# byu-magicc/VI-EKF

Hardware: AMD Instinct MI355X
Metric: EKF steps/sec (IMU-rate propagate + N_feat updates), batch=1024, N_feat=50 (higher is better)
Workload: dtype f64

## Files before the change

### vi_ekf_amd/csrc/viekf_fused_lds.hpp

```cpp
#pragma once
#include <cstddef>

#include "viekf_instance_rows.hpp"

#if defined(__HIPCC__)
#define VIEKF_HD __host__ __device__
#else
#define VIEKF_HD
#endif

namespace viekf {

constexpr int RES_FMT_LOAD_PACKED = 1, RES_FMT_STORE_PACKED = 2, RES_FMT_P_ONLY = 4;
constexpr int launch_pack(bool prop, int kp, int fmt, int dbg) { return (prop ? (1 | (kp << 16)) : 0) | (fmt << 1) | ((dbg & 0xff) << 8); }
constexpr int launch_prop(int w) { return w & 1; }
constexpr int launch_fmt(int w) { return (w >> 1) & 7; }
constexpr int launch_dbg(int w) { return (w >> 8) & 0xff; }
constexpr int launch_kp(int w) { return (w >> 16) > 0 ? (w >> 16) : 1; }

enum : unsigned { SM_RES1 = 1, SM_RES2 = 2, SM_TILE = 4, SM_TILE_PAIR = 8 };
struct SmWords {
  const char* name;
  int at, count;
  bool is_int;
  bool zero;
  unsigned live;
  const char* writer;
  const char* reader;
};

namespace res_sm {
enum { MB_H0, MB_H1, MB_H2, MB_H3, MB_R0, MB_R1, MB_S0, MB_S1, MB_S2, MB_S3, MB_GATE, MB_FIELDS };
constexpr int MB_STRIDE = 16;
constexpr int mbox(int mb) { return MB_STRIDE * mb; }
constexpr int mbox_seq(int mb) { return 32 + mb; }
constexpr int fix_word(int role, int par) { return (role == 2 ? 36 : 40) + par; }
constexpr int DT = 42;
constexpr int nan_word(int role, int phase) { return (role == 2 ? 52 : 44) + phase % 3; }
constexpr int gate_word(int phase) { return 50 + (phase & 1); }
constexpr int CTRL_WORDS = 64;
constexpr int SQRTQU = CTRL_WORDS, QXB = SQRTQU + 6;
constexpr int len(bool staged) { return staged ? QXB + 16 : CTRL_WORDS; }
inline constexpr SmWords kWords[] = {
    {"mailbox 0", mbox(0), MB_FIELDS, false, false, SM_RES2, "the service wave that holds the feature (send)", "the other service wave (recv)"},
    {"mailbox 1", mbox(1), MB_FIELDS, false, false, SM_RES2, "the service wave that holds the feature (send)", "the other service wave (recv)"},
    {"mailbox sequence numbers", mbox_seq(0), 2, true, true, SM_RES2, "send", "recv (polls)"},
    {"fix mailbox non-empty, body wave", fix_word(2, 0), 2, false, true, SM_RES2, "service role 2", "workers (fix_word)"},
    {"fix mailbox non-empty", fix_word(0, 0), 2, false, true, SM_RES1 | SM_RES2, "service role 0 / 1", "workers (fix_word)"},
    {"dt", DT, 1, false, false, SM_RES1 | SM_RES2, "prologue; service (next propagate of several)", "service, res_prop_setup"},
    {"NaN guard", nan_word(0, 0), 3, false, true, SM_RES1 | SM_RES2, "service role 0 / 1 (gain_rows)", "workers; service role 2"},
    {"(dead: once the count of published raw columns)", 49, 1, true, true, 0, "nobody", "nobody"},
    {"gate verdict", gate_word(0), 2, false, true, SM_RES1 | SM_RES2, "service role 0 / 1 (gain_rows)", "workers"},
    {"NaN guard, body wave", nan_word(2, 0), 3, false, true, SM_RES2, "service role 2 (gain_rows)", "workers; service role 1"},
    {"sqrt(Qu)", SQRTQU, 6, false, false, SM_RES1 | SM_RES2, "prologue", "res_prop_setup"},
    {"Qx of the body rows", QXB, 16, false, false, SM_RES1 | SM_RES2, "prologue", "res_prop_body"},
};
}

namespace tile_sm {
enum { MB_G00, MB_G01, MB_G11, MB_SKIP, MB_FIELDS };
constexpr int MB_STRIDE = 8;
constexpr int mbox(int mb) { return MB_STRIDE * mb; }
constexpr int fix_word(int par) { return 40 + par; }
constexpr int DT = 42;
constexpr int nan_word(int phase) { return 44 + phase % 3; }
constexpr int TRIPS = 60;
constexpr int CTRL_WORDS = 64;
constexpr int len() { return CTRL_WORDS; }
inline constexpr SmWords kWords[] = {
    {"mailbox 0", mbox(0), MB_FIELDS, false, false, SM_TILE | SM_TILE_PAIR, "service (publish)", "workers"},
    {"mailbox 1", mbox(1), MB_FIELDS, false, false, SM_TILE | SM_TILE_PAIR, "service (publish)", "workers"},
    {"fix mailbox non-empty", fix_word(0), 2, false, true, SM_TILE | SM_TILE_PAIR, "service", "workers"},
    {"dt", DT, 1, false, false, SM_TILE | SM_TILE_PAIR, "prologue; service (next propagate of several)", "service, res_prop_setup"},
    {"NaN in the column pair", nan_word(0), 3, false, true, SM_TILE | SM_TILE_PAIR, "workers (set; clear two phases ahead)", "workers, service"},
    {"updates that will run", TRIPS, 1, false, false, SM_TILE_PAIR, "prologue", "both halves of a paired workgroup"},
};
}

template <int NWD>
constexpr unsigned long long sm_zero_mask(const SmWords (&words)[NWD]) {
  unsigned long long m = 0;
  for (int i = 0; i < NWD; i++)
    if (words[i].zero)
      for (int w = words[i].at; w < words[i].at + words[i].count; w++) m |= 1ull << w;
  return m;
}

constexpr std::size_t kBodyCtxBytes = 440;
constexpr int ZK = 9;
constexpr int ZS = 26;

VIEKF_HD inline int res_mcap(int N) { return N > 64 ? 80 : 64; }

constexpr bool res_batched_loads(int RB, int NW) { return NW != 7 && RB != 8; }

struct ResLds {
  int xs, Kt, Wt, Praw, lam, sm, fixadd, fixset, Z, phiff, Abb, Gb, Phibb, Mbb, Gdb, Pbb, T16, xdb, ctx, Pbc, PhibbT, Pd, PsiP, Pi, Xi, AvG, Lbc, mslot, mseq, mz, mR, img_len, total;
  VIEKF_HD ResLds(int N, int n, int nxs, bool staged, std::size_t ctx_bytes) {
    const int nf = 3 * N;
    int o = 0;
    auto take = [&](int cnt) { int r = o; o += (cnt + 1) & ~1; return r; };
    xs = take(nxs);
    lam = take(n);
    sm = take(res_sm::len(staged));
    fixadd = take(2 * (N > 0 ? N : 1)); fixset = take(2 * (N > 0 ? N : 1));
    Z = take(nf * ZS > 4 * n ? nf * ZS : 4 * n);
    phiff = take(9 * (N > 0 ? N : 1));
    const int u0 = o;
    Abb = take(256); Gb = take(96); Phibb = take(256); PhibbT = take(256); Gdb = take(96); T16 = take(256);
    PsiP = take(ZK * 16); Pi = take(ZK * ZK); Xi = take(ZK * 16); AvG = take(18);
    const int uprop = o;
    o = u0;
    Kt = take(2 * n); Wt = take(2 * n);
    Praw = take(4 * n > 256 ? 4 * n : 256);
    Pd = take(4 * (N > 0 ? N : 1));
    if (uprop > o) o = uprop;
    img_len = o - Z;
    Mbb = take(256); Pbb = take(256);
    xdb = take(16);
    ctx = take((int)((ctx_bytes + 7) / 8));
    Pbc = take(nf * 16);
    Lbc = take(48);
    const int mc = res_mcap(N);
    mslot = take(mc / 2); mseq = take(mc); mz = take(2 * mc); mR = take(4 * mc);
    total = o;
  }
};

VIEKF_HD inline int tile_nt(int N) { return 1 + (N + 4) / 5; }

struct TileLds {
  int xs, lam, sm, fixadd, fixset, Z, phiff, Abb, Gb, Phibb, PhibbT, Gdb, T16, PsiP, Pi, Xi, AvG, Cb, Eb, Pd, Mbb, Pbb, xdb, ctx, Pbc,
      mslot, mseq, mz, mR, total;
  VIEKF_HD TileLds(int N, int n, int nxs, std::size_t ctx_bytes) {
    const int nf = 3 * N, NQ = 16 * tile_nt(N);
    int o = 0;
    auto take = [&](int cnt) { int r = o; o += (cnt + 1) & ~1; return r; };
    xs = take(nxs);
    lam = take(n);
    sm = take(tile_sm::len());
    fixadd = take(2 * (N > 0 ? N : 1)); fixset = take(2 * (N > 0 ? N : 1));
    Z = take(nf * ZS);
    phiff = take(9 * (N > 0 ? N : 1));
    const int u0 = o;
    Abb = take(256); Gb = take(96); Phibb = take(256); PhibbT = take(256); Gdb = take(96); T16 = take(256);
    PsiP = take(ZK * 16); Pi = take(ZK * ZK); Xi = take(ZK * 16); AvG = take(18);
    const int uprop = o;
    o = u0;
    Cb = take(4 * NQ);
    Eb = take(4 * NQ);
    Pd = take(4 * (N > 0 ? N : 1));
    if (uprop > o) o = uprop;
    Mbb = take(256); Pbb = take(256);
    xdb = take(16);
    ctx = take((int)((ctx_bytes + 7) / 8));
    Pbc = take(nf * 16);
    const int mc = res_mcap(N);
    mslot = take(mc / 2); mseq = take(mc); mz = take(2 * mc); mR = take(4 * mc);
    total = o;
  }
  VIEKF_HD int pair_word(int half, int w) const { return half * total + sm + w; }
};

}
```

### vi_ekf_amd/csrc/viekf_host.hpp

```cpp
#pragma once
#include <map>
#include <string>
#include <vector>

namespace viekf {

typedef std::map<std::string, std::string> YamlMap;
bool yaml_parse_file(const std::string& path, YamlMap& out, std::string& err);
bool yaml_get_doubles(const YamlMap& m, const std::string& key, double* out, int count, std::string& err);
bool yaml_get_string(const YamlMap& m, const std::string& key, std::string& out, std::string& err);
int set_last_error(int code, const std::string& msg);
bool build_resmap(int N, int RB, int NWV, std::vector<int>& map, int* used_slots = nullptr);

inline int cov_ld(int num_features) {
  const int n = 16 + 3 * num_features;
#ifdef VIEKF_LD_PAD_ALL
  return (n + 15) & ~15;
#endif
  return num_features > 77 ? (n + 15) & ~15 : (n + 1) & ~1;
}

}
```

### vi_ekf_amd/csrc/viekf_resident_worker.hpp

```cpp
#pragma once
#include "viekf_resident_prop.hpp"

namespace viekf {


struct StoreChunk { int f0, f1, rb, h; };
__device__ __forceinline__ bool store_chunk_at(int f0, int N, int n, int img_len, StoreChunk& c) {
  if (f0 >= N) return false;
  c.f0 = f0;
  c.rb = (16 + 3 * f0) & ~1;
  c.h = ((n + 1) & ~1) - c.rb;
  c.f1 = min(N, f0 + max(1, img_len / (3 * c.h)));
  return true;
}
template <int T>
__device__ __forceinline__ void res_store_chunk(const StreamArgs& a, const ResShared& S, const StoreChunk& c, int tid) {
  const int n = S.n, ld = a.ld;
  double* P = a.P_out + S.so * n * ld;
  const double* img = S.Z;
  const int ncol = 3 * (c.f1 - c.f0), lane = tid & 63, w = tid >> 6;
  constexpr int NWV = T / 64;
  if ((n & 1) == 0) {
#pragma unroll 2
    for (int col = w; col < ncol; col += NWV) {
      const int j = 16 + 3 * c.f0 + col;
      const double* src = img + col * c.h - c.rb;
      for (int i0 = c.rb; i0 < n; i0 += 256) {
        double2 v[2];
#pragma unroll
        for (int u = 0; u < 2; u++) v[u] = lds_ld2(src + min(i0 + 2 * (lane + 64 * u), n - 2));
#pragma unroll
        for (int u = 0; u < 2; u++) {
          const int i = i0 + 2 * (lane + 64 * u);
          if (i < n && i + 1 >= j) *reinterpret_cast<double2*>(P + i + (long)j * ld) = v[u];
        }
      }
    }
  } else {
#pragma unroll 2
    for (int col = w; col < ncol; col += NWV) {
      const int j = 16 + 3 * c.f0 + col;
      const double* src = img + col * c.h - c.rb;
      for (int i = c.rb + lane; i < n; i += 64)
        if (i >= j) P[i + (long)j * ld] = src[i];
    }
  }
}

template <int RB, int TW>
__device__ __forceinline__ void res_store_packed(double* img, const double (&pb)[RB][9], const double* Pbc, const double* Pbb,
                                                 int N, int t) {
  constexpr ResPack K(0, RB, TW / 64);
  v2f64* dst = reinterpret_cast<v2f64*>(img) + t;
#pragma unroll
  for (int p = 0; p < K.npair; p++) {
    v2f64 v;
    v.x = pb[(2 * p) / 9][(2 * p) % 9];
    v.y = pb[(2 * p + 1) / 9][(2 * p + 1) % 9];
    dst[p * TW] = v;
  }
  if ((9 * RB) & 1) img[K.single + t] = pb[RB - 1][8];
  v2f64* gc = reinterpret_cast<v2f64*>(img + K.pbc);
  for (int e = t; e < 24 * N; e += TW) gc[e] = *reinterpret_cast<const v2f64*>(Pbc + 2 * e);
  v2f64* gb = reinterpret_cast<v2f64*>(img + K.pbc + 48 * N);
  for (int e = t; e < 128; e += TW) gb[e] = *reinterpret_cast<const v2f64*>(Pbb + 2 * e);
}
__device__ __forceinline__ void res_body_items(const ResShared& S, const double* kP, bool run, int id, int nthreads,
                                               int first, int last, int slot2, double* rawdst) {
  const double* wP = kP + 2 * S.n;
  double* Pbc = S.Pbc;
  const int j2 = ((first + id) & 7) * 2;
  double2 cw0 = {}, cw1 = {}, cl[3] = {};
  if (run) {
    cw0 = lds_ld2(wP + 2 * j2);
    cw1 = lds_ld2(wP + 2 * j2 + 2);
#pragma unroll
    for (int q = 0; q < 3; q++) cl[q] = lds_ld2(S.Lbc + 16 * q + j2);
  }
#pragma unroll 1
  for (int item = first + id; item < last; item += nthreads) {
    const int g = item >> 3;
    double2 cpv[3];
#pragma unroll
    for (int q = 0; q < 3; q++) cpv[q] = lds_ld2(Pbc + (3 * g + q) * 16 + j2);
    if (run) {
      double2 cki[3];
#pragma unroll
      for (int q = 0; q < 3; q++) cki[q] = lds_ld2(kP + 2 * (16 + 3 * g + q));
#pragma unroll
      for (int q = 0; q < 3; q++) {
        cpv[q].x = fma(-cl[q].x, fma(cki[q].y, cw0.y, cki[q].x * cw0.x), cpv[q].x);
        cpv[q].y = fma(-cl[q].y, fma(cki[q].y, cw1.y, cki[q].x * cw1.x), cpv[q].y);
        *reinterpret_cast<double2*>(Pbc + (3 * g + q) * 16 + j2) = cpv[q];
      }
    }
    if (g == slot2) {
      double* st = rawdst + 2 * j2;
      *reinterpret_cast<double2*>(st) = make_double2(cpv[0].x, cpv[1].x);
      *reinterpret_cast<double2*>(st + 2) = make_double2(cpv[0].y, cpv[1].y);
    }
  }
}
template <int RB, int TW, bool MP, int T = TW + 64, bool ZU = false, bool BL = true>
__device__ __forceinline__ void res_worker(const StreamArgs& a, const ResShared& S, int tid) {
  constexpr bool SU = res_setup_under_load(RB, TW / 64, MP);
  constexpr int RR = res_rotating_reads(RB, TW / 64, MP, ZU);
  const int N = S.N, n = S.n, ld = a.ld, nf = S.nf, len = S.len;
  double* P = a.P + S.si * n * ld;
  const int tid_ = tid;
  constexpr int NWV = TW / 64;
  const DevParams& prm = a.prm(uniform_filter(S.b));
  double* Pbc = S.Pbc;
  double* Pbb = S.Pbb;
  const int* __restrict__ resmap = a.resmap;
  auto blk = [&](const int (&w)[RB], int t, int ia, int& I, int& J) -> bool {
    return res_word_blk(BL ? w[ia] : resmap[ia * TW + t], I, J);
  };
  const bool own_diag = tid_ < N;

  double pb[RB][9];
  const bool ldp = (S.fmt & RES_FMT_LOAD_PACKED) != 0;
  double Lff[9];
  bool partial_su = false;
  if (SU) {
    const double lf[3] = {a.lam(uniform_filter(S.b))[16], a.lam(uniform_filter(S.b))[17], a.lam(uniform_filter(S.b))[18]};
#pragma unroll
    for (int r = 0; r < 3; r++)
#pragma unroll
      for (int s = 0; s < 3; s++) Lff[r * 3 + s] = uniform_f64(prm.use_partial_update ? (lf[s] + lf[r] - lf[r] * lf[s]) : 1.0);
    partial_su = prm.use_partial_update != 0;
  }
  if (ldp) {
    const int t = opaque(tid_);
    constexpr ResPack K(0, RB, TW / 64);
    const v2f64* gc = reinterpret_cast<const v2f64*>(P + K.pbc);
    for (int e = t; e < 24 * N; e += TW) *reinterpret_cast<v2f64*>(Pbc + 2 * e) = gc[e];
    const v2f64* gb = reinterpret_cast<const v2f64*>(P + K.pbc + 48 * N);
    for (int e = t; e < 128; e += TW) *reinterpret_cast<v2f64*>(Pbb + 2 * e) = gb[e];
  }
  if (SU) {
    for (int e = tid; !ldp && e < nf * 16; e += TW) {
      const int k = e / nf, row = e - k * nf;
      Pbc[row * 16 + k] = P[(16 + row) + (long)k * ld];
    }
    for (int e = tid; !ldp && e < 256; e += TW) {
      const int r = e & 15, c = e >> 4;
      Pbb[r * 16 + c] = P[max(r, c) + (long)min(r, c) * ld];
    }
  }
  int ws[SU ? RB : 1];
  double qs[3];
  {
    const int tq = opaque(tid_);
    int ew[RB];
    if (BL) res_words<RB, TW>(resmap, tq, ew);
    if (SU) {
#pragma unroll
      for (int ia = 0; ia < RB; ia++) ws[ia] = ew[ia];
      if (S.do_prop) {
#pragma unroll
        for (int r = 0; r < 3; r++) qs[r] = a.qx(uniform_filter(S.b))[16 + 3 * min(tq, N - 1) + r];
      }
    }
#pragma unroll
    for (int ia = 0; ia < (SU ? RB / 4 : RB); ia++) {
      int I, J;
      blk(ew, tq, ia, I, J);
      const bool up = I < J;
      const int br = 16 + 3 * (up ? J : I), bc = 16 + 3 * (up ? I : J);
      const unsigned cbase = (unsigned)(br + bc * ld);
      const unsigned base = ldp ? 2u * (unsigned)tq : cbase, base1 = ldp ? (unsigned)tq : cbase;
#pragma unroll
      for (int s = 0; s < 3; s++)
#pragma unroll
        for (int r = 0; r < 3; r++) {
          const int rr = (I == J) ? max(r, s) : (up ? s : r), cc = (I == J) ? min(r, s) : (up ? r : s);
          constexpr ResPack K(0, RB, TW / 64);
          const int q = ia * 9 + r * 3 + s;
          const unsigned offp = (unsigned)K.elem(q, 0), offc = (unsigned)(rr + cc * ld);
          pb[ia][r * 3 + s] = P[((q < 2 * K.npair) ? base : base1) + (ldp ? offp : offc)];
        }
    }
    for (int e = tid; !SU && !ldp && e < nf * 16; e += TW) {
      const int k = e / nf, row = e - k * nf;
      Pbc[row * 16 + k] = P[(16 + row) + (long)k * ld];
    }
    for (int e = tid; !SU && !ldp && e < 256; e += TW) {
      const int r = e & 15, c = e >> 4;
      Pbb[r * 16 + c] = P[max(r, c) + (long)min(r, c) * ld];
    }
  }

  auto issue_chunk = [&](auto kc) {
    constexpr int k = decltype(kc)::value + 1, lo = RB * k / 4, hi = RB * (k + 1) / 4;
    const int tq = opaque(tid_);
#pragma unroll
    for (int ia = lo; ia < hi; ia++) {
      int I, J;
      res_word_blk(ws[SU ? ia : 0], I, J);
      const bool up = I < J;
      const int br = 16 + 3 * (up ? J : I), bc = 16 + 3 * (up ? I : J);
      const unsigned cbase = (unsigned)(br + bc * ld);
      const unsigned base = ldp ? 2u * (unsigned)tq : cbase, base1 = ldp ? (unsigned)tq : cbase;
#pragma unroll
      for (int s = 0; s < 3; s++)
#pragma unroll
        for (int r = 0; r < 3; r++) {
          const int rr = (I == J) ? max(r, s) : (up ? s : r), cc = (I == J) ? min(r, s) : (up ? r : s);
          constexpr ResPack K(0, RB, TW / 64);
          const int q = ia * 9 + r * 3 + s;
          const unsigned offp = (unsigned)K.elem(q, 0), offc = (unsigned)(rr + cc * ld);
          pb[ia][r * 3 + s] = P[((q < 2 * K.npair) ? base : base1) + (ldp ? offp : offc)];
        }
    }
  };

  auto sym_diag = [&]() {
    if (own_diag) { pb[0][3] = pb[0][1]; pb[0][6] = pb[0][2]; pb[0][7] = pb[0][5]; }
  };
  if (!SU) {
    sym_diag();
    const double lf[3] = {a.lam(uniform_filter(S.b))[16], a.lam(uniform_filter(S.b))[17], a.lam(uniform_filter(S.b))[18]};
#pragma unroll
    for (int r = 0; r < 3; r++)
#pragma unroll
      for (int s = 0; s < 3; s++) Lff[r * 3 + s] = uniform_f64(prm.use_partial_update ? (lf[s] + lf[r] - lf[r] * lf[s]) : 1.0);
  }
  const bool partial = SU ? partial_su : prm.use_partial_update != 0;
  int par = 0;
  constexpr int NSV = (T - TW) / 64;
  auto fix_word = [&](int mb) -> double { return (NSV > 1) ? S.sm[res_sm::fix_word(1, mb)] + S.sm[res_sm::fix_word(2, mb)] : S.sm[res_sm::fix_word(0, mb)]; };
  RES_STAMP(S, tid == 0, 64);
  __syncthreads();
  RES_STAMP(S, tid == 0, 65);

  const int nkp = MP ? S.kp : 1;
  int eu[RB];
  if (S.do_prop)
   for (int kp = 0; kp < nkp; kp++) {
    const int tk = MP ? opaque(tid) : tid;
    const double* Z = S.Z; double* phiff = S.phiff;
    int ep[RB];
    double qd[3];
    if (SU) {
#pragma unroll
      for (int ia = 0; ia < RB; ia++) ep[ia] = ws[SU ? ia : 0];
#pragma unroll
      for (int r = 0; r < 3; r++) qd[r] = qs[r];
    } else if (BL) {
      const int tq = opaque(tid_);
      res_words<RB, TW>(resmap, tq, ep);
#pragma unroll
      for (int r = 0; r < 3; r++) qd[r] = a.qx(uniform_filter(S.b))[16 + 3 * min(tq, N - 1) + r];
    }
    if (MP || !BL) res_prop_setup<TW>(a, S, tk);
    else if (SU) res_prop_setup<TW, true, decltype(issue_chunk), res_service_setup(RB, TW / 64, MP)>(a, S, tk, issue_chunk);
    else res_prop_setup<TW, true>(a, S, tk);
    RES_STAMP(S, tid == 0, 66);
    __syncthreads();
    RES_STAMP(S, tid == 0, 67);
#ifdef VIEKF_STAMPS
    asm volatile("s_waitcnt vmcnt(0)" ::: "memory");
#endif
    RES_STAMP(S, tid == 0, 74);
    if (SU) sym_diag();

#pragma unroll
    for (int ia = 0; ia < RB; ia++) {
      const int tq = BL ? 0 : opaque(tid_);
      int I, J;
      const bool v = blk(ep, tq, ia, I, J);
      const double* fj = phiff + 9 * J;
#pragma unroll
      for (int r = 0; r < 3; r++) {
        const double p0 = pb[ia][r * 3 + 0], p1 = pb[ia][r * 3 + 1], p2 = pb[ia][r * 3 + 2];
#pragma unroll
        for (int s = 0; s < 3; s++) pb[ia][r * 3 + s] = p0 * fj[s * 3 + 0] + p1 * fj[s * 3 + 1] + p2 * fj[s * 3 + 2];
      }
      const double* fi = phiff + 9 * I;
#pragma unroll
      for (int s = 0; s < 3; s++) {
        const double p0 = pb[ia][0 * 3 + s], p1 = pb[ia][1 * 3 + s], p2 = pb[ia][2 * 3 + s];
#pragma unroll
        for (int r = 0; r < 3; r++) pb[ia][r * 3 + s] = fi[r * 3 + 0] * p0 + fi[r * 3 + 1] * p1 + fi[r * 3 + 2] * p2;
      }
      if (BL) {
        if (ia == 0 && own_diag) { pb[0][0] += qd[0]; pb[0][4] += qd[1]; pb[0][8] += qd[2]; }
      } else if (v && I == J) {
        pb[ia][0] += a.qx(uniform_filter(S.b))[16 + 3 * I + 0];
        pb[ia][4] += a.qx(uniform_filter(S.b))[16 + 3 * I + 1];
        pb[ia][8] += a.qx(uniform_filter(S.b))[16 + 3 * I + 2];
      }
      __builtin_amdgcn_sched_barrier(0);
      if (RB > 4) {
#pragma unroll
        for (int e = 0; e < 9; e++) asm volatile("" : "+v"(pb[ia][e]));
      }
      group_fence<(RB > 4)>();
    }
    RES_STAMP(S, tid == 0, 68);
    int zoff[RB];
    {
      const int tq = BL ? 0 : opaque(tid_);
#pragma unroll
      for (int ia = 0; ia < RB; ia++) {
        int I, J;
        blk(ep, tq, ia, I, J);
        zoff[ia] = (3 * I * ZS) | ((3 * J * ZS) << 16);
      }
    }
    auto contract = [&](int k, auto crossed) {
      constexpr bool CROSS = decltype(crossed)::value;
      if (RR & 2) {
        double2 xb[2][3], yb[2][3];
#pragma unroll
        for (int ia = 0; ia < 2; ia++) {
          const double* zi = Z + (zoff[ia] & 0xffff) + 2 * k;
          const double* zj = Z + (zoff[ia] >> 16) + 2 * k;
#pragma unroll
          for (int r = 0; r < 3; r++) xb[ia][r] = lds_ld2(zi + r * ZS);
#pragma unroll
          for (int s = 0; s < 3; s++) yb[ia][s] = lds_ld2(zj + s * ZS);
        }
#pragma unroll
        for (int ia = 0; ia < RB; ia++) {
          const int ib = ia & 1;
#pragma unroll
          for (int r = 0; r < 3; r++)
#pragma unroll
            for (int s = 0; s < 3; s++) {
              double acc = pb[ia][r * 3 + s];
              acc = fma(xb[ib][r].x, CROSS ? yb[ib][s].y : yb[ib][s].x, acc);
              acc = fma(xb[ib][r].y, CROSS ? yb[ib][s].x : yb[ib][s].y, acc);
              pb[ia][r * 3 + s] = acc;
            }
          group_fence<true>();
          if (ia + 2 < RB) {
            constexpr int RBL = RB - 1;
            const int in = (ia + 2 < RB) ? ia + 2 : RBL;
            const double* zi = Z + (zoff[in] & 0xffff) + 2 * k;
            const double* zj = Z + (zoff[in] >> 16) + 2 * k;
#pragma unroll
            for (int r = 0; r < 3; r++) xb[ib][r] = lds_ld2(zi + r * ZS);
#pragma unroll
            for (int s = 0; s < 3; s++) yb[ib][s] = lds_ld2(zj + s * ZS);
          }
        }
        return;
      }
#pragma unroll
      for (int ia = 0; ia < RB; ia++) {
        const double* zi = Z + (zoff[ia] & 0xffff) + 2 * k;
        const double* zj = Z + (zoff[ia] >> 16) + 2 * k;
        double2 xv[3], yv[3];
#pragma unroll
        for (int r = 0; r < 3; r++) xv[r] = lds_ld2(zi + r * ZS);
#pragma unroll
        for (int s = 0; s < 3; s++) yv[s] = lds_ld2(zj + s * ZS);
#pragma unroll
        for (int r = 0; r < 3; r++)
#pragma unroll
          for (int s = 0; s < 3; s++) {
            double acc = pb[ia][r * 3 + s];
            acc = fma(xv[r].x, CROSS ? yv[s].y : yv[s].x, acc);
            acc = fma(xv[r].y, CROSS ? yv[s].x : yv[s].y, acc);
            pb[ia][r * 3 + s] = acc;
          }
        if (ia & 1) group_fence<(RB > 4)>();
      }
    };
#pragma unroll 1
    for (int k = 0; k < ZK; k++) contract(k, std::true_type{});
#pragma unroll 1
    for (int k = ZK; k < ZK + 3; k++) contract(k, std::false_type{});
    sym_diag();
    RES_STAMP(S, tid == 0, 69);
    if (BL && !MP) res_words<RB, TW>(resmap, opaque(tid_), eu);
    if (MP) res_prop_body<TW, BL>(a, S, tk);
    par ^= 1;
    RES_STAMP(S, tid == 0, 70);
    __syncthreads();
    for (int e = tk; e < 256; e += TW) { const int r = e >> 4, c = e & 15; Pbb[e] = S.Mbb[min(r, c) * 16 + max(r, c)]; }
    if (MP && kp + 1 < nkp && own_diag && tid_ < len && fix_word(par ^ 1) != 0.0) {
      const int mb = par ^ 1, I = tid_;
      const double ad = S.fixadd[mb * N + I], st = S.fixset[mb * N + I];
      if (ad != 0.0) { pb[0][8] += ad; S.fixadd[mb * N + I] = 0.0; }
      if (st != 0.0) { pb[0][8] = prm.P0_feat[2]; S.fixset[mb * N + I] = 0.0; }
    }
   }

  if (SU && !S.do_prop) {
    issue_chunk(std::integral_constant<int, 0>{});
    issue_chunk(std::integral_constant<int, 1>{});
    issue_chunk(std::integral_constant<int, 2>{});
    sym_diag();
  }
  int Ib[RB], Jb[RB];
  bool vb[RB];
  if (BL && (MP || !S.do_prop)) res_words<RB, TW>(resmap, opaque(tid_), eu);
#pragma unroll
  for (int ia = 0; ia < RB; ia++) vb[ia] = blk(eu, tid_, ia, Ib[ia], Jb[ia]);
  const double p0rr = uniform_f64(prm.P0_feat[2]);
  auto bb_mask = [&](int r, int c) -> double { const double lr_ = S.lam[r], lc_ = S.lam[c]; return partial ? (lc_ + lr_ - lr_ * lc_) : 1.0; };
  double bbL0 = 1.0, bbL1 = 1.0;
  {
    constexpr int BBT0 = (TW >= 128) ? 128 : TW;
    const int ib0 = tid - (TW - BBT0);
    if (ib0 >= 0 && ib0 < 128) { bbL0 = bb_mask(ib0 >> 3, (ib0 & 7) * 2); bbL1 = bb_mask(ib0 >> 3, (ib0 & 7) * 2 + 1); }
  }
  auto apply_fixes = [&](int mb, double pending) {
    if (pending == 0.0) return;
    if (own_diag && tid_ < len) {
      VIEKF_COLD_BEGIN();
      const int I = tid_;
      const double ad = S.fixadd[mb * N + I], st = S.fixset[mb * N + I];
      if (ad != 0.0) { pb[0][8] += ad; S.fixadd[mb * N + I] = 0.0; }
      if (st != 0.0) { pb[0][8] = p0rr; S.fixset[mb * N + I] = 0.0; }
      VIEKF_COLD_END();
    }
  };
  auto extract_cols = [&](int slot, double* Pw) {
#pragma unroll
    for (int ia = 0; ia < RB; ia++) {
      const int I = Ib[ia], J = Jb[ia];
      const bool asrow = J == slot;
      const bool ascol = !asrow && I == slot;
      if (vb[ia] && (asrow || ascol)) {
        const int base = 16 + 3 * (asrow ? I : J);
        const double a0 = pb[ia][0], a1 = asrow ? pb[ia][1] : pb[ia][3];
        const double b0 = asrow ? pb[ia][3] : pb[ia][1], b1 = pb[ia][4];
        const double c0 = asrow ? pb[ia][6] : pb[ia][2], c1 = asrow ? pb[ia][7] : pb[ia][5];
        *reinterpret_cast<double2*>(Pw + 2 * (base + 0)) = make_double2(a0, a1);
        *reinterpret_cast<double2*>(Pw + 2 * (base + 1)) = make_double2(b0, b1);
        *reinterpret_cast<double2*>(Pw + 2 * (base + 2)) = make_double2(c0, c1);
      }
    }
  };

  int m = res_next_valid(S, 0);
  if (own_diag) {
    *reinterpret_cast<double2*>(S.Pd + 4 * tid_) = make_double2(pb[0][0], pb[0][1]);
    *reinterpret_cast<double2*>(S.Pd + 4 * tid_ + 2) = make_double2(pb[0][3], pb[0][4]);
  }
  int2 sq = S.mseq[min(m, S.mcap - 1)];
  if (m < S.M) {
    apply_fixes(par ^ 1, fix_word(par ^ 1));
    const int s0 = S.mslot[m];
    extract_cols(s0, S.Praw);
    if (sq.y >= 0) extract_cols(sq.y, S.Praw + 2 * n);
    const int e = opaque(tid);
    if (e < 16) {
      const int sf = (e < 8) ? s0 : sq.y, ijj = (e & 7) * 2;
      if (sf >= 0) {
        const double2 q0 = lds_ld2(Pbc + (3 * sf) * 16 + ijj);
        const double2 q1 = lds_ld2(Pbc + (3 * sf + 1) * 16 + ijj);
        double* d = S.Praw + ((e < 8) ? 0 : 2 * n) + 2 * ijj;
        *reinterpret_cast<double2*>(d) = make_double2(q0.x, q1.x);
        *reinterpret_cast<double2*>(d + 2) = make_double2(q0.y, q1.y);
      }
    }
  }
  RES_STAMP(S, tid == 0, 71);
  __syncthreads();
  __syncthreads();
  int it_ = 0;
  int cnt = 0;
  while (m < S.M) {
    const int mnext = sq.x;
    RES_MARK("worker.phase_top");
    const double* kP = (cnt & 1) ? S.Z : S.Kt;
    const double* wP = kP + 2 * n;
    __builtin_amdgcn_s_setprio(1);
    const double fixpending = fix_word(par ^ 1);
    const double gflag = S.sm[res_sm::gate_word(cnt)];
    const double nanw = (NSV > 1) ? S.sm[res_sm::nan_word(1, cnt)] + S.sm[res_sm::nan_word(2, cnt)] : S.sm[res_sm::nan_word(0, cnt)];
    sq = S.mseq[min(mnext, S.mcap - 1)];
    RES_STAMP(S, tid == 0 && it_ < 8, 80 + 4 * it_ + 1);
    RES_STAMP(S, (tid & 63) == 0 && it_ == 3, 192 + 4 * (tid >> 6) + 0);
    const int it = tid;
    constexpr int GB = (RB <= 4) ? RB : 2;
    RES_MARK("worker.block_sweep");
    const bool gated = gflag != 0.0;
    const bool run = !gated && nanw == 0.0 && !RES_ABLATE(S, 1);
    bool fixed = false;
    if (RR & 1) {
      apply_fixes(par ^ 1, fixpending);
      if (run) {
        double2 kb[2][3], wb[2][3];
#pragma unroll
        for (int ia = 0; ia < 2; ia++) {
#pragma unroll
          for (int r = 0; r < 3; r++) kb[ia][r] = lds_ld2(kP + 2 * (16 + 3 * Ib[ia] + r));
#pragma unroll
          for (int s = 0; s < 3; s++) wb[ia][s] = lds_ld2(wP + 2 * (16 + 3 * Jb[ia] + s));
        }
#pragma unroll
        for (int ia = 0; ia < RB; ia++) {
          const int ib = ia & 1;
#pragma unroll
          for (int r = 0; r < 3; r++)
#pragma unroll
            for (int s = 0; s < 3; s++) {
              if (ZU && !(r == 2 && s == 2)) {
                pb[ia][r * 3 + s] = fma(-kb[ib][r].y, wb[ib][s].y, fma(-kb[ib][r].x, wb[ib][s].x, pb[ia][r * 3 + s]));
              } else {
                const double t = fma(kb[ib][r].y, wb[ib][s].y, kb[ib][r].x * wb[ib][s].x);
                pb[ia][r * 3 + s] = fma(-Lff[r * 3 + s], t, pb[ia][r * 3 + s]);
              }
            }
          group_fence<true>();
          if (ia + 2 < RB) {
            constexpr int RBL = RB - 1;
            const int in = (ia + 2 < RB) ? ia + 2 : RBL;
#pragma unroll
            for (int r = 0; r < 3; r++) kb[ib][r] = lds_ld2(kP + 2 * (16 + 3 * Ib[in] + r));
#pragma unroll
            for (int s = 0; s < 3; s++) wb[ib][s] = lds_ld2(wP + 2 * (16 + 3 * Jb[in] + s));
          }
        }
      }
    } else
#pragma unroll
    for (int g0 = 0; g0 < RB; g0 += GB) {
      double2 kI[GB][3], wJ[GB][3];
#pragma unroll
      for (int ig = 0; ig < GB; ig++) {
        const int ia = (g0 + ig < RB) ? g0 + ig : RB - 1;
#pragma unroll
        for (int r = 0; r < 3; r++) kI[ig][r] = lds_ld2(kP + 2 * (16 + 3 * Ib[ia] + r));
#pragma unroll
        for (int s = 0; s < 3; s++) wJ[ig][s] = lds_ld2(wP + 2 * (16 + 3 * Jb[ia] + s));
      }
      if (!fixed) { apply_fixes(par ^ 1, fixpending); fixed = true; }
      if (run) {
#pragma unroll
        for (int ig = 0; ig < GB; ig++) {
          if (g0 + ig >= RB) continue;
          const int ia = g0 + ig;
#pragma unroll
          for (int r = 0; r < 3; r++)
#pragma unroll
            for (int s = 0; s < 3; s++) {
              if (ZU && !(r == 2 && s == 2)) {
                pb[ia][r * 3 + s] = fma(-kI[ig][r].y, wJ[ig][s].y, fma(-kI[ig][r].x, wJ[ig][s].x, pb[ia][r * 3 + s]));
              } else {
                const double t = fma(kI[ig][r].y, wJ[ig][s].y, kI[ig][r].x * wJ[ig][s].x);
                pb[ia][r * 3 + s] = fma(-Lff[r * 3 + s], t, pb[ia][r * 3 + s]);
              }
            }
        }
      }
      group_fence<(RB > GB)>();
    }
    sym_diag();
    RES_MARK("worker.column_extraction");
    RES_STAMP(S, tid == 0 && it_ < 8, 160 + 4 * it_ + 0);
    double* rawdst = S.Praw + (cnt & 1) * 2 * n;
    if (sq.y >= 0 && !RES_ABLATE(S, 4) && !(RES_ABLATE(S, 8) && (cnt & 1))) extract_cols(sq.y, rawdst);
    __builtin_amdgcn_s_setprio(0);
    RES_STAMP(S, tid == 0 && it_ < 8, 160 + 4 * it_ + 1);
    RES_STAMP(S, (tid & 63) == 0 && it_ == 3, 192 + 4 * (tid >> 6) + 2);
    __builtin_amdgcn_sched_barrier(0);
    RES_MARK("worker.body_items");
    res_body_items(S, kP, run, (it >= 64) ? it - 64 : it + TW - 64, TW, 0, 8 * N, sq.y, rawdst);
    RES_MARK("worker.body_block");
    if (run) {
      constexpr int BBT = (TW >= 128) ? 128 : TW;
#pragma unroll
      for (int ib = it - (TW - BBT); ib >= 0 && ib < 128; ib += BBT) {
        const int br = ib >> 3, bc2 = (ib & 7) * 2;
        double2 bpv = *reinterpret_cast<double2*>(Pbb + br * 16 + bc2);
        const double2 kr = lds_ld2(kP + 2 * br), wr = lds_ld2(wP + 2 * br);
        const double2 k0 = lds_ld2(kP + 2 * bc2), w0 = lds_ld2(wP + 2 * bc2);
        const double2 k1 = lds_ld2(kP + 2 * bc2 + 2), w1 = lds_ld2(wP + 2 * bc2 + 2);
        const double L0 = (BBT == 128) ? bbL0 : bb_mask(br, bc2), L1 = (BBT == 128) ? bbL1 : bb_mask(br, bc2 + 1);
        const bool up0 = br <= bc2, up1 = br <= bc2 + 1;
        const double2 ka = up0 ? kr : k0, wa = up0 ? w0 : wr;
        const double2 kb = up1 ? kr : k1, wb = up1 ? w1 : wr;
        bpv.x = fma(-L0, fma(ka.y, wa.y, ka.x * wa.x), bpv.x);
        bpv.y = fma(-L1, fma(kb.y, wb.y, kb.x * wb.x), bpv.y);
        *reinterpret_cast<double2*>(Pbb + br * 16 + bc2) = bpv;
      }
    }
    RES_MARK("worker.phase_tail");
    par ^= 1;
    cnt++;
    RES_STAMP(S, tid == 0 && it_ < 8, 80 + 4 * it_ + 2);
    RES_STAMP(S, (tid & 63) == 0 && it_ == 3, 192 + 4 * (tid >> 6) + 1);
    __syncthreads();
    RES_STAMP(S, tid == 0 && it_ < 8, 80 + 4 * it_ + 3);
    RES_STAMP(S, (tid & 63) == 0 && it_ == 3, 192 + 4 * (tid >> 6) + 3);
    it_++;
    m = mnext;
  }
  RES_MARK("worker.loop_end");
  apply_fixes(par ^ 1, fix_word(par ^ 1));
  RES_STAMP(S, tid == 0, 72);
  __syncthreads();

  P = a.P_out + S.so * n * ld;
  if (S.fmt & RES_FMT_STORE_PACKED) {
    res_store_packed<RB, TW>(P, pb, Pbc, Pbb, N, opaque(tid_));
  } else {
    int es[RB];
    if (BL) res_words<RB, TW>(resmap, opaque(tid_), es);
    for (int e = opaque(tid); e < nf * 16; e += TW) {
      const int k = e / nf, row = e - k * nf;
      P[(16 + row) + (long)k * ld] = Pbc[row * 16 + k];
    }
    for (int e = opaque(tid); e < 256; e += TW) P[(e >> 4) + (long)(e & 15) * ld] = Pbb[e];
    double* img = S.Z;
    const int gtid = threadIdx.x;
    RES_STAMP(S, tid == 0, 224);
    StoreChunk sc;
    int ch = 0;
    for (int f0 = 0; store_chunk_at(f0, N, n, S.img_len, sc); f0 = sc.f1, ch++) {
      const int f1 = sc.f1;
      const int tq = BL ? 0 : opaque(tid_);
#pragma unroll
      for (int ia = 0; ia < RB; ia++) {
        int I, J;
        if (blk(es, tq, ia, I, J)) {
          if (I >= J && J >= f0 && J < f1) {
            double* d = img + (3 * (J - f0)) * sc.h + (16 + 3 * I - sc.rb);
#pragma unroll
            for (int s = 0; s < 3; s++)
#pragma unroll
              for (int r = 0; r < 3; r++) d[s * sc.h + r] = pb[ia][r * 3 + s];
          }
          if (I < J && I >= f0 && I < f1) {
            double* d = img + (3 * (I - f0)) * sc.h + (16 + 3 * J - sc.rb);
#pragma unroll
            for (int r = 0; r < 3; r++)
#pragma unroll
              for (int s = 0; s < 3; s++) d[r * sc.h + s] = pb[ia][r * 3 + s];
          }
        }
      }
      RES_STAMP(S, tid == 0 && ch < 3, 225 + 4 * ch);
      __syncthreads();
      RES_STAMP(S, tid == 0 && ch < 3, 226 + 4 * ch);
      res_store_chunk<T>(a, S, sc, gtid);
      RES_STAMP(S, tid == 0 && ch < 3, 227 + 4 * ch);
      __syncthreads();
      RES_STAMP(S, tid == 0 && ch < 3, 228 + 4 * ch);
    }
  }
  RES_STAMP(S, tid == 0, 73);
}


}
```

### vi_ekf_amd/csrc/viekf_resmap.cpp

```cpp
#include <algorithm>
#include <cstdint>
#include <utility>
#include <vector>

#include "viekf_host.hpp"
#include "viekf_instance_rows.hpp"

bool viekf::build_resmap(int N, int RB, int NWV, std::vector<int>& map, int* used_slots) {
  const int TW = 64 * NWV;
  map.assign((size_t)RB * TW, 0);
  if (N > TW || N > 255) return false;
  auto put = [&](int slot, int t, int I, int J) { map[(size_t)slot * TW + t] = I | (J << 8) | (1 << 16); };
  for (int t = 0; t < N; t++) put(0, t, t, t);
  struct Group { int slot, wave; std::vector<int> free_lanes; };
  std::vector<Group> groups;
  for (int s = 0; s < RB; s++)
    for (int w = 0; w < NWV; w++) {
      Group g{s, w, {}};
      for (int l = 0; l < 64; l++)
        if (!(s == 0 && 64 * w + l < N)) g.free_lanes.push_back(l);
      groups.push_back(g);
    }
  typedef std::vector<std::pair<int, int>> Unit;
  std::vector<Unit> ragged;
  const int kf = N / 8, r = N % 8;
  for (int TI = 0; TI < kf; TI++)
    for (int TJ = 0; TJ < TI; TJ++) {
      const int pref = (TI + TJ) % NWV;
      int best = -1, bestkey = 1 << 30;
      for (int g = 0; g < (int)groups.size(); g++) {
        if (groups[g].free_lanes.size() != 64) continue;
        const int key = ((groups[g].wave - pref + NWV) % NWV) * 64 + groups[g].slot;
        if (key < bestkey) { bestkey = key; best = g; }
      }
      if (best < 0) {
        Unit u;
        for (int i = 0; i < 8; i++)
          for (int j = 0; j < 8; j++) u.push_back({8 * TI + i, 8 * TJ + j});
        ragged.push_back(u);
        continue;
      }
      for (int i = 0; i < 8; i++)
        for (int j = 0; j < 8; j++) put(groups[best].slot, 64 * groups[best].wave + 8 * i + j, 8 * TI + i, 8 * TJ + j);
      groups[best].free_lanes.clear();
    }
  for (int TD = 0; TD < kf; TD++) {
    Unit u;
    for (int i = 0; i < 8; i++)
      for (int j = 0; j < i; j++) u.push_back({8 * TD + i, 8 * TD + j});
    ragged.push_back(u);
  }
  if (r) {
    for (int TJ = 0; TJ < kf; TJ++) {
      Unit u;
      for (int i = 0; i < r; i++)
        for (int j = 0; j < 8; j++) u.push_back({8 * kf + i, 8 * TJ + j});
      ragged.push_back(u);
    }
    Unit u;
    for (int i = 0; i < r; i++)
      for (int j = 0; j < i; j++) u.push_back({8 * kf + i, 8 * kf + j});
    if (!u.empty()) ragged.push_back(u);
  }
  std::stable_sort(ragged.begin(), ragged.end(), [](const Unit& x, const Unit& y) { return x.size() > y.size(); });
  for (const Unit& u : ragged) {
    int best = -1;
    size_t bestslack = ~(size_t)0;
    for (int g = 0; g < (int)groups.size(); g++) {
      const size_t f = groups[g].free_lanes.size();
      if (f >= u.size() && f - u.size() < bestslack) { bestslack = f - u.size(); best = g; }
    }
    size_t k = 0;
    if (best >= 0) {
      Group& G = groups[best];
      for (; k < u.size(); k++) { put(G.slot, 64 * G.wave + G.free_lanes.front(), u[k].first, u[k].second); G.free_lanes.erase(G.free_lanes.begin()); }
      continue;
    }
    while (k < u.size()) {
      int big = -1;
      for (int g = 0; g < (int)groups.size(); g++)
        if (!groups[g].free_lanes.empty() && (big < 0 || groups[g].free_lanes.size() > groups[big].free_lanes.size())) big = g;
      if (big < 0) return false;
      Group& G = groups[big];
      while (k < u.size() && !G.free_lanes.empty()) {
        put(G.slot, 64 * G.wave + G.free_lanes.front(), u[k].first, u[k].second);
        G.free_lanes.erase(G.free_lanes.begin());
        k++;
      }
    }
  }
  if (N <= 128) {
    typedef unsigned __int128 fmask_t;
    const int ng = RB * NWV;
    std::vector<fmask_t> mask(ng, (fmask_t)0);
    auto remask = [&](int g) {
      fmask_t mk = 0;
      const int slot = g / NWV, wave = g % NWV;
      for (int l = 0; l < 64; l++) {
        const int e = map[(size_t)slot * TW + 64 * wave + l];
        if (e >> 16) mk |= ((fmask_t)1 << (e & 0xff)) | ((fmask_t)1 << ((e >> 8) & 0xff));
      }
      mask[g] = mk;
    };
    for (int g = 0; g < ng; g++) remask(g);
    struct Cost { long mx, summx, sq; bool operator<(const Cost& o) const { return mx != o.mx ? mx < o.mx : (summx != o.summx ? summx < o.summx : sq < o.sq); } };
    auto cost = [&]() {
      Cost c{0, 0, 0};
      for (int f = 0; f < N; f++) {
        long fm = 0;
        for (int w = 0; w < NWV; w++) {
          long cnt = 0;
          for (int sl = 0; sl < RB; sl++) cnt += (long)((mask[sl * NWV + w] >> f) & 1);
          fm = std::max(fm, cnt);
          c.sq += cnt * cnt;
        }
        c.mx = std::max(c.mx, fm);
        c.summx += fm;
      }
      return c;
    };
    auto whole = [&](int g) { return !(g / NWV == 0 && 64 * (g % NWV) < N); };
    Cost best = cost();
    for (bool improved = true; improved;) {
      improved = false;
      for (int g1 = 0; g1 < ng; g1++)
        for (int g2 = g1 + 1; g2 < ng; g2++) {
          if (!whole(g1) || !whole(g2) || g1 % NWV == g2 % NWV) continue;
          std::swap(mask[g1], mask[g2]);
          const Cost c = cost();
          if (c < best) {
            best = c;
            improved = true;
            int* p1 = &map[(size_t)(g1 / NWV) * TW + 64 * (g1 % NWV)];
            int* p2 = &map[(size_t)(g2 / NWV) * TW + 64 * (g2 % NWV)];
            for (int l = 0; l < 64; l++) std::swap(p1[l], p2[l]);
          } else {
            std::swap(mask[g1], mask[g2]);
          }
        }
    }
  }
  int used = 1;
  for (int w = 0; w < NWV; w++) {
    int dst = (64 * w < N) ? 1 : 0;
    for (int sl = dst; sl < RB; sl++) {
      bool any = false;
      for (int l = 0; l < 64 && !any; l++) any = (map[(size_t)sl * TW + 64 * w + l] >> 16) != 0;
      if (!any) continue;
      if (sl != dst)
        for (int l = 0; l < 64; l++) std::swap(map[(size_t)sl * TW + 64 * w + l], map[(size_t)dst * TW + 64 * w + l]);
      dst++;
    }
    used = std::max(used, dst);
  }
  if (used_slots) *used_slots = used;
  return true;
}

extern "C" {

int viekf_debug_build_resmap(int n_feat, int rb, int nw, int32_t* out) {
  std::vector<int> map;
  int used = 0;
  if (n_feat < 1 || rb < 1 || nw < 1 || !out) return -1;
  if (n_feat * (n_feat + 1) / 2 > rb * nw * 64 || !viekf::build_resmap(n_feat, rb, nw, map, &used)) return -1;
  for (size_t i = 0; i < map.size(); i++) out[i] = map[i];
  return used;
}

int viekf_debug_res_instance(int i, int* rb, int* nw, int* nmin, int* nmax) {
  if (i < 0 || i >= viekf::kNumResInst || !rb || !nw || !nmin || !nmax) return -1;
  const viekf::ResInst& r = viekf::kResInst[i];
  *rb = r.RB; *nw = r.NW; *nmin = r.nmin; *nmax = r.nmax;
  return 0;
}

int viekf_debug_packed_layout(int n_feat, int rb, int nw, int32_t* elem, int32_t* info) {
  if (n_feat < 1 || rb < 1 || nw < 1 || !elem || !info) return -1;
  const viekf::ResPack K(n_feat, rb, nw);
  for (int q = 0; q < 9 * rb; q++)
    for (int t = 0; t < K.TW; t++) elem[(size_t)q * K.TW + t] = K.elem(q, t);
  const int n = 16 + 3 * n_feat, ld = viekf::cov_ld(n_feat);
  info[0] = K.pbc; info[1] = K.pbb; info[2] = K.total; info[3] = n * ld; info[4] = K.fits(n, ld) ? 1 : 0;
  return 0;
}

}
```

Measured before the change: 3.513 million.

## Reassign resident-map lanes to cut repeated feature slots and merge column publishes

```diff
diff --git a/vi_ekf_amd/csrc/viekf_fused_lds.hpp b/vi_ekf_amd/csrc/viekf_fused_lds.hpp
--- a/vi_ekf_amd/csrc/viekf_fused_lds.hpp
+++ b/vi_ekf_amd/csrc/viekf_fused_lds.hpp
@@ -94,6 +94,11 @@
 
 constexpr bool res_batched_loads(int RB, int NW) { return NW != 7 && RB != 8; }
 
+#ifndef VIEKF_MERGED_PUBLISH
+#define VIEKF_MERGED_PUBLISH 1
+#endif
+constexpr bool res_merged_publish(int RB, int NW, bool MP) { return (VIEKF_MERGED_PUBLISH) != 0 && !MP && RB == 7 && NW == 3; }
+
 struct ResLds {
   int xs, Kt, Wt, Praw, lam, sm, fixadd, fixset, Z, phiff, Abb, Gb, Phibb, Mbb, Gdb, Pbb, T16, xdb, ctx, Pbc, PhibbT, Pd, PsiP, Pi, Xi, AvG, Lbc, mslot, mseq, mz, mR, img_len, total;
   VIEKF_HD ResLds(int N, int n, int nxs, bool staged, std::size_t ctx_bytes) {
diff --git a/vi_ekf_amd/csrc/viekf_host.hpp b/vi_ekf_amd/csrc/viekf_host.hpp
--- a/vi_ekf_amd/csrc/viekf_host.hpp
+++ b/vi_ekf_amd/csrc/viekf_host.hpp
@@ -11,6 +11,8 @@
 bool yaml_get_string(const YamlMap& m, const std::string& key, std::string& out, std::string& err);
 int set_last_error(int code, const std::string& msg);
 bool build_resmap(int N, int RB, int NWV, std::vector<int>& map, int* used_slots = nullptr);
+int resmap_wave_repeats(const std::vector<int>& map, int RB, int NWV, int w);
+std::vector<int> resmap_assign(const std::vector<std::vector<long>>& cost);
 
 inline int cov_ld(int num_features) {
   const int n = 16 + 3 * num_features;
diff --git a/vi_ekf_amd/csrc/viekf_resident_worker.hpp b/vi_ekf_amd/csrc/viekf_resident_worker.hpp
--- a/vi_ekf_amd/csrc/viekf_resident_worker.hpp
+++ b/vi_ekf_amd/csrc/viekf_resident_worker.hpp
@@ -105,6 +105,7 @@
 __device__ __forceinline__ void res_worker(const StreamArgs& a, const ResShared& S, int tid) {
   constexpr bool SU = res_setup_under_load(RB, TW / 64, MP);
   constexpr int RR = res_rotating_reads(RB, TW / 64, MP, ZU);
+  constexpr bool MG = res_merged_publish(RB, TW / 64, MP);
   const int N = S.N, n = S.n, ld = a.ld, nf = S.nf, len = S.len;
   double* P = a.P + S.si * n * ld;
   const int tid_ = tid;
@@ -420,6 +421,38 @@
     }
   };
   auto extract_cols = [&](int slot, double* Pw) {
+    if (MG) {
+      double a0 = 0.0, a1 = 0.0, b0 = 0.0, b1 = 0.0, c0 = 0.0, c1 = 0.0;
+      int base = 0;
+      bool matched = false;
+#pragma unroll
+      for (int ia = 0; ia < RB; ia++) {
+        const int I = Ib[ia], J = Jb[ia];
+        const bool asrow = J == slot;
+        const bool ascol = !asrow && I == slot;
+        if (vb[ia] && (asrow || ascol)) {
+          const int bs = 16 + 3 * (asrow ? I : J);
+          const double x0 = pb[ia][0], x1 = asrow ? pb[ia][1] : pb[ia][3];
+          const double y0 = asrow ? pb[ia][3] : pb[ia][1], y1 = pb[ia][4];
+          const double z0 = asrow ? pb[ia][6] : pb[ia][2], z1 = asrow ? pb[ia][7] : pb[ia][5];
+          if (!matched) {
+            a0 = x0; a1 = x1; b0 = y0; b1 = y1; c0 = z0; c1 = z1;
+            base = bs;
+            matched = true;
+          } else {
+            *reinterpret_cast<double2*>(Pw + 2 * (bs + 0)) = make_double2(x0, x1);
+            *reinterpret_cast<double2*>(Pw + 2 * (bs + 1)) = make_double2(y0, y1);
+            *reinterpret_cast<double2*>(Pw + 2 * (bs + 2)) = make_double2(z0, z1);
+          }
+        }
+      }
+      if (matched) {
+        *reinterpret_cast<double2*>(Pw + 2 * (base + 0)) = make_double2(a0, a1);
+        *reinterpret_cast<double2*>(Pw + 2 * (base + 1)) = make_double2(b0, b1);
+        *reinterpret_cast<double2*>(Pw + 2 * (base + 2)) = make_double2(c0, c1);
+      }
+      return;
+    }
 #pragma unroll
     for (int ia = 0; ia < RB; ia++) {
       const int I = Ib[ia], J = Jb[ia];
diff --git a/vi_ekf_amd/csrc/viekf_resmap.cpp b/vi_ekf_amd/csrc/viekf_resmap.cpp
--- a/vi_ekf_amd/csrc/viekf_resmap.cpp
+++ b/vi_ekf_amd/csrc/viekf_resmap.cpp
@@ -154,7 +154,93 @@
     used = std::max(used, dst);
   }
   if (used_slots) *used_slots = used;
+  for (int w = 0; w < NWV; w++)
+    for (int round = 0, before = resmap_wave_repeats(map, RB, NWV, w); before > 0 && round < 8; round++) {
+      for (int sl = 0; sl < used; sl++) {
+        std::vector<int> lanes;
+        for (int l = 0; l < 64; l++)
+          if (!(sl == 0 && 64 * w + l < N)) lanes.push_back(l);
+        const int m = (int)lanes.size();
+        if (m < 2) continue;
+        std::vector<std::vector<unsigned char>> cnt(m, std::vector<unsigned char>(256, 0));
+        for (int q = 0; q < m; q++)
+          for (int s2 = 0; s2 < RB; s2++) {
+            const int e = map[(size_t)s2 * TW + 64 * w + lanes[q]];
+            if (s2 == sl || !(e >> 16)) continue;
+            cnt[q][e & 0xff]++;
+            if (((e >> 8) & 0xff) != (e & 0xff)) cnt[q][(e >> 8) & 0xff]++;
+          }
+        std::vector<int> ent(m);
+        for (int p = 0; p < m; p++) ent[p] = map[(size_t)sl * TW + 64 * w + lanes[p]];
+        std::vector<std::vector<long>> cost(m, std::vector<long>(m, 0));
+        for (int p = 0; p < m; p++)
+          for (int q = 0; q < m; q++) {
+            long c = 0;
+            if (ent[p] >> 16) c = (cnt[q][ent[p] & 0xff] ? 1 : 0) + (cnt[q][(ent[p] >> 8) & 0xff] ? 1 : 0);
+            cost[p][q] = c * 1024 + (p != q ? 1 : 0);
+          }
+        const std::vector<int> to = resmap_assign(cost);
+        for (int p = 0; p < m; p++) map[(size_t)sl * TW + 64 * w + lanes[to[p]]] = ent[p];
+      }
+      const int after = resmap_wave_repeats(map, RB, NWV, w);
+      if (after >= before) break;
+      before = after;
+    }
   return true;
+}
+
+int viekf::resmap_wave_repeats(const std::vector<int>& map, int RB, int NWV, int w) {
+  const int TW = 64 * NWV;
+  int rep = 0;
+  for (int l = 0; l < 64; l++) {
+    int cnt[256] = {0};
+    for (int sl = 0; sl < RB; sl++) {
+      const int e = map[(size_t)sl * TW + 64 * w + l];
+      if (!(e >> 16)) continue;
+      const int I = e & 0xff, J = (e >> 8) & 0xff;
+      if (cnt[I]++) rep++;
+      if (J != I && cnt[J]++) rep++;
+    }
+  }
+  return rep;
+}
+
+std::vector<int> viekf::resmap_assign(const std::vector<std::vector<long>>& cost) {
+  const int m = (int)cost.size();
+  const long INF = 1L << 60;
+  std::vector<long> u(m + 1, 0), v(m + 1, 0);
+  std::vector<int> p(m + 1, 0), way(m + 1, 0);
+  for (int i = 1; i <= m; i++) {
+    p[0] = i;
+    int j0 = 0;
+    std::vector<long> minv(m + 1, INF);
+    std::vector<char> usedc(m + 1, 0);
+    do {
+      usedc[j0] = 1;
+      const int i0 = p[j0];
+      long delta = INF;
+      int j1 = 0;
+      for (int j = 1; j <= m; j++) {
+        if (usedc[j]) continue;
+        const long cur = cost[i0 - 1][j - 1] - u[i0] - v[j];
+        if (cur < minv[j]) { minv[j] = cur; way[j] = j0; }
+        if (minv[j] < delta) { delta = minv[j]; j1 = j; }
+      }
+      for (int j = 0; j <= m; j++) {
+        if (usedc[j]) { u[p[j]] += delta; v[j] -= delta; }
+        else minv[j] -= delta;
+      }
+      j0 = j1;
+    } while (p[j0] != 0);
+    do {
+      const int j1 = way[j0];
+      p[j0] = p[j1];
+      j0 = j1;
+    } while (j0);
+  }
+  std::vector<int> to(m, 0);
+  for (int j = 1; j <= m; j++) to[p[j] - 1] = j - 1;
+  return to;
 }
 
 extern "C" {
@@ -166,6 +252,15 @@
   if (n_feat * (n_feat + 1) / 2 > rb * nw * 64 || !viekf::build_resmap(n_feat, rb, nw, map, &used)) return -1;
   for (size_t i = 0; i < map.size(); i++) out[i] = map[i];
   return used;
+}
+
+int viekf_debug_resmap_repeats(int n_feat, int rb, int nw, int32_t* out) {
+  std::vector<int> map;
+  if (n_feat < 1 || rb < 1 || nw < 1 || !out) return -1;
+  if (n_feat * (n_feat + 1) / 2 > rb * nw * 64 || !viekf::build_resmap(n_feat, rb, nw, map)) return -1;
+  int sum = 0;
+  for (int w = 0; w < nw; w++) sum += out[w] = viekf::resmap_wave_repeats(map, rb, nw, w);
+  return sum;
 }
 
 int viekf_debug_res_instance(int i, int* rb, int* nw, int* nmin, int* nmax) {
```

Result: faster. 3.550 million (median of 6 runs) (+1.1%).
